# StuLiu/RegDA

Measured on AMD Instinct MI355X. Metric: src+tgt 512x512 image-pairs/sec (SSL step), higher is better.
Workload: dtype bf16; 1 GPU; st.regda.2potsdam SSL step, resnet101 DeepLabV2(PPM), batch 8+8 512x512 per GPU, online EMA teacher; global_batch=8, parallelism=dp1

## Files before the change

include/rgda_hip.h:

```cpp
#ifndef RGDA_HIP_H
#define RGDA_HIP_H

#include <stddef.h>
#include <stdint.h>

#ifdef __cplusplus
extern "C" {
#endif

#define RGDA_ABI_VERSION 10
#define RGDA_STAT_REPLICAS 8
#define RGDA_STAT_FRAC_FWD 26
#define RGDA_STAT_FRAC_BWD 40
typedef int64_t rgda_stat_t;
#define RGDA_LAYOUT_TILE 64

typedef void* rgda_stream_t;

enum rgda_status {
    RGDA_OK = 0,
    RGDA_ERR_ARG = -1,
    RGDA_ERR_WORKSPACE = -2,
    RGDA_ERR_LAUNCH = -3,
    RGDA_ERR_UNSUPPORTED = -4
// ... 138 lines not shown
    int lddw, co_split;
} rgda_wgrad_desc;
size_t rgda_conv2d_wgrad_workspace(const rgda_wgrad_desc* descs, int n);
const char* rgda_conv2d_wgrad_kernel(const rgda_wgrad_desc* desc);
int rgda_conv2d_wgrad_grouped(const rgda_wgrad_desc* descs, int n, void* ws, size_t ws_bytes, rgda_stream_t stream);

int rgda_stem_im2col(const float* img, void* col, int N, int H, int W, int Ho, int Wo, int Kp,
                     rgda_stream_t stream);

int rgda_stem_conv(const float* img, const void* wgt, void* y, int ldy, rgda_stat_t* stats, int stat_groups, int N,
                   int H, int W, int Ho, int Wo, rgda_stream_t stream);
int rgda_stem_conv_bneval(const float* img, const void* wgt, void* y, int ldy, const float* running_mean,
                          const float* running_var, const float* gamma, const float* beta, float eps, int relu,
                          int N, int H, int W, int Ho, int Wo, rgda_stream_t stream);

int rgda_bn_stats(const void* x, int ldx, rgda_stat_t* stats, int64_t M, int C, rgda_stream_t stream);
int rgda_bn_finalize(const rgda_stat_t* stats, float* mi, float* running_mean, float* running_var,
                     int64_t* num_batches_tracked, int64_t M, int C, int groups, float eps,
                     float momentum, rgda_stream_t stream);
int rgda_bn_apply(const void* x, int ldx, const float* mi, const float* gamma, const float* beta,
                  const void* res, int ldres, const float* nscale, int rows_per_image, void* y,
                  int ldy, int64_t M, int C, int relu, int groups, rgda_stream_t stream);
int rgda_bn_train_apply(const void* x, int ldx, const rgda_stat_t* stats, float* mi, float* running_mean,
                        float* running_var, int64_t* num_batches_tracked, const float* gamma,
                        const float* beta, const void* res, int ldres, const float* nscale,
                        int rows_per_image, void* y, int ldy, uint8_t* relu_mask, int64_t M, int C, int relu,
                        int groups, float eps, float momentum, rgda_stream_t stream);
int rgda_bn_bwd_reduce(const void* g, int ldg, const void* y, int ldy, const uint8_t* relu_mask, const void* x,
                       int ldx, const float* mi, const float* nscale, int rows_per_image, rgda_stat_t* sums,
                       int64_t M, int C, int relu, const float* gamma, const float* beta, int groups,
                       rgda_stream_t stream);
int rgda_bn_bwd_apply(const void* g, int ldg, const void* y, int ldy, const uint8_t* relu_mask, const void* x,
                      int ldx, const float* mi, const float* gamma, const float* nscale,
                      int rows_per_image, const rgda_stat_t* sums, void* dx, int lddx, void* gmask,
                      int ldgm, float* dgamma, float* dbeta, int64_t M, int C, int relu, const float* beta,
                      void* act_out, int ldact, int groups, rgda_stream_t stream);

typedef struct rgda_bn_small_fwd_desc {
    const void* x; void* y; uint8_t* relu_mask; const float* gamma; const float* beta; float* mi;
    float* running_mean; float* running_var; int64_t* num_batches_tracked;
    int64_t M; int ldx, ldy, C, groups, relu; float eps, momentum;
} rgda_bn_small_fwd_desc;
typedef struct rgda_bn_small_bwd_desc {
    const void* g; const void* y; const uint8_t* relu_mask; const void* x; void* dx; const float* mi; const float* gamma;
    float* dgamma; float* dbeta;
    int64_t M; int ldg, ldy, ldx, lddx, C, groups, relu;
} rgda_bn_small_bwd_desc;
int rgda_bn_train_small(const rgda_bn_small_fwd_desc* descs, int n, rgda_stream_t stream);
int rgda_bn_bwd_small(const rgda_bn_small_bwd_desc* descs, int n, rgda_stream_t stream);

int rgda_maxpool_fwd(const void* x, void* y, uint8_t* idx, int N, int H, int W, int C, int Ho,
                     int Wo, rgda_stream_t stream);
int rgda_maxpool_bwd(const void* gy, const uint8_t* idx, void* gx, int N, int H, int W, int C,
                     int Ho, int Wo, rgda_stream_t stream);
int rgda_maxpool_fwd_bnin(const rgda_bn_operand* bn_in, const void* x, void* y, uint8_t* idx, int N, int H, int W,
                          int C, int Ho, int Wo, rgda_stream_t stream);

int rgda_instnorm_fwd(const void* x, int ldx, void* y0, void* y1, int ldy, float* feat_nchw,
                      float* mi, int N, int HW, int C, float eps, rgda_stream_t stream);
int rgda_instnorm_bwd(const void* ga, const void* gb, int ldg, const void* gc, int ldgc,
                      const void* x, int ldx, const float* mi, void* dx, int lddx, int N, int HW,
                      int C, rgda_stream_t stream);

int rgda_spatial_mix(const void* in, int ldin, const float* Mx, void* out, int ldout, int N, int I,
                     int J, int C, int accumulate, int out_f32, rgda_stream_t stream);

int rgda_spatial_mix_multi(int nsrc, const void* const* ins, const int* ldins, const float* const* mats,
                           const int* Js, void* out, int ldout, int N, int I, int C, rgda_stream_t stream);

int rgda_classifier_fwd(const void* hidden, int ldh, const float* w, const float* bias,
                        float* logits, int N, int HW, int C, int ncls, rgda_stream_t stream);
size_t rgda_classifier_bwd_workspace(int64_t M, int C, int ncls);
int rgda_classifier_bwd(const void* hidden, int ldh, const float* w, const float* glogits,
                        void* dhidden, int lddh, float* dw, float* db, int N, int HW, int C,
                        int ncls, void* ws, size_t ws_bytes, rgda_stream_t stream);


int rgda_sumsq(const float* g, int64_t n, float* out, float* ws, rgda_stream_t stream);

int rgda_sgd_step(float* p, const float* g, float* v, float* shadow, void* p_bf16, void* shadow_bf16,
                  const float* gnorm_sq, const float* lr_dev, int64_t n, float momentum,
                  float weight_decay, float max_norm, float gscale, float ema_decay,
                  int first_step, rgda_stream_t stream);

size_t rgda_stem_wgrad_workspace(int N, int H, int W);
int rgda_stem_wgrad(const float* img, const void* dy, int lddy, float* dw, void* ws, size_t ws_bytes, int N, int H,
                    int W, int Ho, int Wo, rgda_stream_t stream);

int rgda_weight_transpose_bf16(const float* w, void* wt, int Co, int T, int Ci, rgda_stream_t stream);
int rgda_weight_transpose_batched(const int64_t* table, int n, int64_t total_blocks, rgda_stream_t stream);
int rgda_cast_bf16(const float* src, void* dst, int64_t n, rgda_stream_t stream);
int rgda_cast_f32(const void* src_bf16, float* dst, int64_t n, rgda_stream_t stream);
int rgda_ddp_accumulate_bf16(const void* recv, int world, void* out, int64_t shard_elems, rgda_stream_t stream);

typedef void* rgda_comm_t;
#define RGDA_COMM_ID_BYTES 128
#define RGDA_COMM_F32 0
#define RGDA_COMM_BF16 1
#define RGDA_COMM_I64 2
#define RGDA_COMM_F64 3
int rgda_comm_unique_id(void* id_128_bytes);
int rgda_comm_init(const void* id_128_bytes, int rank, int world, rgda_comm_t* comm);
int rgda_comm_destroy(rgda_comm_t comm);
int rgda_comm_all_reduce(rgda_comm_t comm, void* buf, int64_t n, int dtype, rgda_stream_t stream);
int rgda_comm_all_gather(rgda_comm_t comm, const void* send, void* recv, int64_t n_per_rank, int dtype,
                         rgda_stream_t stream);
int rgda_comm_all_to_all(rgda_comm_t comm, const void* send, void* recv, int64_t n_per_rank, int dtype,
                         rgda_stream_t stream);
int rgda_pad_cast_bf16(const float* src, void* dst, int R, int K, int Kp, rgda_stream_t stream);
int rgda_unpad_acc_f32(const float* src, float* dst, int R, int K, int Kp, rgda_stream_t stream);
int rgda_fill_zero(void* p, size_t bytes, rgda_stream_t stream);
int rgda_copy_multi(int n, void* const* dsts, const void* const* srcs, const size_t* bytes, rgda_stream_t stream);
int rgda_set_f32(float* p, float value, rgda_stream_t stream);
int rgda_dropout_mask(float* out, int64_t n, float p, uint64_t seed, rgda_stream_t stream);
int rgda_add_bf16(const void* a, int lda, const void* b, int ldb, void* out, int ldo, int64_t M,
                  int C, rgda_stream_t stream);


int rgda_dihedral_nchw(const float* src, float* dst, int N, int C, int Hs, int Ws, int hflip, int rot_k,
                       int flip_first, float scale, int accumulate, rgda_stream_t stream);

int rgda_pad_rows_nchw(const float* src, float* dst, int N, int C, int h, int w, int top, int bottom,
                       rgda_stream_t stream);
int rgda_window_crop(const float* full, float* tile, int N, int C, int Hf, int Wf, int y1, int x1, int h, int w,
                     int Th, int Tw, rgda_stream_t stream);
int rgda_window_accumulate(const float* tile, float* full, float* count, int N, int C, int Hf, int Wf, int y1,
                           int x1, int h, int w, int Th, int Tw, rgda_stream_t stream);
int rgda_window_normalise(float* full, const float* count, int N, int C, int Hf, int Wf, rgda_stream_t stream);

int rgda_window_gather(const float* src_f32, const uint8_t* src_u8, const float* lut, const int32_t* windows, int K,
                       int views, int n, int C, int H, int W, int Th, int Tw, float* out, int* flag,
                       rgda_stream_t stream);
int rgda_window_scatter(const float* pred, const int32_t* windows, int K, int views, int n, int C, int H, int W, int Th,
                        int Tw, int row0, int rows, float* full, float* count, int* flag, rgda_stream_t stream);
int rgda_window_finish(float* full, const float* count, int n, int C, int H, int W, uint8_t* labels_u8,
                       int64_t* labels_i64, const int64_t* y_true, int64_t* cm, int* flag, rgda_stream_t stream);

int rgda_resize_bilinear_ac(const float* src, float* dst, int N, int C, int h, int w, int H, int W,
                            rgda_stream_t stream);


int rgda_augment_tiles(const uint8_t* img, const uint8_t* label, const float* soft, const int32_t* regs,
                       const int32_t* params, int N, int Hi, int Wi, int C, int Ho, int Wo, const float* lut,
                       const int32_t* label_lut, float* img_out, int64_t* label_out, float* soft_out, int64_t* regs_out,
                       int* flag, rgda_stream_t stream);


size_t rgda_superpixels_workspace(int N, int H, int W, int S);
int rgda_superpixels(const uint8_t* img, int N, int H, int W, int S, int m, int iters, int min_area, int32_t* regs_out,
                     int32_t* count_out, void* ws, size_t ws_bytes, rgda_stream_t stream);

int rgda_region_shrink(const int32_t* regs, int N, int H, int W, int win, int fill, int32_t* out, rgda_stream_t stream);


int rgda_argmax_nchw(const float* probs, int64_t* out, int N, int C, int64_t HW, rgda_stream_t stream);
int rgda_confusion_accumulate(const int64_t* y_true, const int64_t* y_pred, int64_t* cm, int* flag, int64_t n,
                              int C, rgda_stream_t stream);


size_t rgda_pcl_loss_workspace(int C, int K);
int rgda_pcl_loss(const float* feat, const int64_t* labels, const float* protos, float* loss, void* dfeat,
                  int lddf, int accumulate, int b, int K, int C, int h, int w, int ignore_label,
                  float temperature, float weight, void* ws, size_t ws_bytes, rgda_stream_t stream);

size_t rgda_coral_loss_workspace(int ns, int nt, int d);
int rgda_coral_loss(const float* feat_s, int bs, int hws, int64_t ldcs, int64_t ldbs,
// ... 36 lines not shown
```

regda_amd/csrc/optim_kernels.hip:

```cpp
#include "common.h"

__global__ void __launch_bounds__(256) sumsq_partial_kernel(const float* __restrict__ g, long long n, float* part) {
    double acc = 0.0;
    long long n4 = n >> 2;
    const float4* g4 = (const float4*)g;
    for (long long i = (long long)blockIdx.x * 256 + threadIdx.x; i < n4; i += (long long)gridDim.x * 256) {
        float4 v = g4[i];
        acc += (double)(v.x * v.x + v.y * v.y) + (double)(v.z * v.z + v.w * v.w);
    }
    if (blockIdx.x == 0 && threadIdx.x < (n & 3)) { float v = g[(n4 << 2) + threadIdx.x]; acc += (double)v * v; }
    __shared__ double red[256];
    red[threadIdx.x] = acc;
    __syncthreads();
    for (int o = 128; o > 0; o >>= 1) {
        if (threadIdx.x < o) red[threadIdx.x] += red[threadIdx.x + o];
        __syncthreads();
    }
    if (threadIdx.x == 0) part[blockIdx.x] = (float)red[0];
}
__global__ void __launch_bounds__(256) sumsq_final_kernel(const float* __restrict__ part, int n, float* out) {
    __shared__ double red[256];
    double acc = 0.0;
    for (int i = threadIdx.x; i < n; i += 256) acc += part[i];
    red[threadIdx.x] = acc;
    __syncthreads();
    for (int o = 128; o > 0; o >>= 1) {
        if (threadIdx.x < o) red[threadIdx.x] += red[threadIdx.x + o];
        __syncthreads();
    }
    if (threadIdx.x == 0) out[0] = (float)red[0];
}

extern "C" int rgda_sumsq(const float* g, int64_t n, float* out, float* ws, rgda_stream_t stream) {
    if (!g || !out || !ws || n <= 0) return RGDA_ERR_ARG;
    hipStream_t st = to_stream(stream);
    int blocks = min(cdiv(n, 256 * 16), 1024);
    sumsq_partial_kernel<<<blocks, 256, 0, st>>>(g, n, ws);
    RGDA_CHECK_LAUNCH();
    sumsq_final_kernel<<<1, 256, 0, st>>>(ws, blocks, out);
    RGDA_CHECK_LAUNCH();
    return RGDA_OK;
}

__global__ void __launch_bounds__(256) sgd_step_kernel(float* __restrict__ p, const float* __restrict__ g,
                                                       float* __restrict__ v, float* __restrict__ shadow,
                                                       bf16_t* __restrict__ pb, bf16_t* __restrict__ sb,
                                                       const float* __restrict__ gnorm_sq,
                                                       const float* __restrict__ lr_dev, long long n4, float momentum,
                                                       float wd, float max_norm, float gscale, float ema_d,
                                                       int first_step) {
    const float total = sqrtf(gnorm_sq[0]) * gscale;
    const float coef = fminf(max_norm / (total + 1e-6f), 1.f) * gscale;
    const float lr = lr_dev[0];
    float4* p4 = (float4*)p;
    const float4* g4 = (const float4*)g;
    float4* v4 = (float4*)v;
    float4* s4 = (float4*)shadow;
    for (long long i = (long long)blockIdx.x * 256 + threadIdx.x; i < n4; i += (long long)gridDim.x * 256) {
        float4 pp = p4[i], gg = g4[i], vv;
        float d0 = gg.x * coef + wd * pp.x, d1 = gg.y * coef + wd * pp.y, d2 = gg.z * coef + wd * pp.z,
              d3 = gg.w * coef + wd * pp.w;
        if (first_step) { vv = make_float4(d0, d1, d2, d3); }
        else {
            vv = v4[i];
            vv.x = momentum * vv.x + d0; vv.y = momentum * vv.y + d1; vv.z = momentum * vv.z + d2; vv.w = momentum * vv.w + d3;
        }
        pp.x -= lr * vv.x; pp.y -= lr * vv.y; pp.z -= lr * vv.z; pp.w -= lr * vv.w;
        v4[i] = vv;
        p4[i] = pp;
        if (shadow) {
            float4 ss = s4[i];
            const float a = 1.f - ema_d;
            ss.x = a * pp.x + ema_d * ss.x; ss.y = a * pp.y + ema_d * ss.y; ss.z = a * pp.z + ema_d * ss.z; ss.w = a * pp.w + ema_d * ss.w;
            s4[i] = ss;
            if (sb) {
                uint2 pk;
                pk.x = pack2bf(ss.x, ss.y);
                pk.y = pack2bf(ss.z, ss.w);
                *(uint2*)(sb + (i << 2)) = pk;
            }
        }
        if (pb) {
            uint2 pk;
            pk.x = pack2bf(pp.x, pp.y);
            pk.y = pack2bf(pp.z, pp.w);
            *(uint2*)(pb + (i << 2)) = pk;
        }
    }
}

extern "C" int rgda_sgd_step(float* p, const float* g, float* v, float* shadow, void* p_bf16, void* shadow_bf16, const float* gnorm_sq,
                             const float* lr_dev, int64_t n, float momentum, float weight_decay, float max_norm,
                             float gscale, float ema_decay, int first_step, rgda_stream_t stream) {
    if (!p || !g || !v || !gnorm_sq || !lr_dev || n <= 0 || (n & 3)) return RGDA_ERR_ARG;
    long long n4 = n >> 2;
    int blocks = min(cdiv(n4, 256 * 4), 4096);
    sgd_step_kernel<<<blocks, 256, 0, to_stream(stream)>>>(p, g, v, shadow, (bf16_t*)p_bf16, (bf16_t*)shadow_bf16, gnorm_sq, lr_dev, n4,
                                                            momentum, weight_decay, max_norm, gscale, ema_decay,
                                                            first_step);
    RGDA_CHECK_LAUNCH();
    return RGDA_OK;
}

__global__ void __launch_bounds__(256) cast_bf16_kernel(const float* __restrict__ src, bf16_t* __restrict__ dst, long long n) {
    long long n4 = n >> 2;
    const float4* s4 = (const float4*)src;
    for (long long i = (long long)blockIdx.x * 256 + threadIdx.x; i < n4; i += (long long)gridDim.x * 256) {
        float4 v = s4[i];
        uint2 pk;
        pk.x = pack2bf(v.x, v.y);
        pk.y = pack2bf(v.z, v.w);
        *(uint2*)(dst + (i << 2)) = pk;
    }
    if (blockIdx.x == 0 && threadIdx.x < (n & 3)) dst[(n4 << 2) + threadIdx.x] = f2bf(src[(n4 << 2) + threadIdx.x]);
}

extern "C" int rgda_cast_bf16(const float* src, void* dst, int64_t n, rgda_stream_t stream) {
    if (!src || !dst || n <= 0) return RGDA_ERR_ARG;
    int blocks = min(cdiv(n, 256 * 16), 4096);
    cast_bf16_kernel<<<blocks, 256, 0, to_stream(stream)>>>(src, (bf16_t*)dst, n);
    RGDA_CHECK_LAUNCH();
    return RGDA_OK;
}

__global__ void __launch_bounds__(256) ddp_accumulate_bf16_kernel(const bf16_t* __restrict__ recv, int world, bf16_t* __restrict__ out,
                                                                  long long s) {
    const long long nv = s >> 3;
    for (long long i = (long long)blockIdx.x * 256 + threadIdx.x; i < nv; i += (long long)gridDim.x * 256) {
        float acc[8] = {0.f, 0.f, 0.f, 0.f, 0.f, 0.f, 0.f, 0.f};
        for (int r = 0; r < world; ++r) {
            const u16x8 v = *(const u16x8*)(recv + (size_t)r * s + i * 8);
#pragma unroll
            for (int e = 0; e < 8; ++e) acc[e] += bf2f(v[e]);
        }
        uint4 pk;
        pk.x = pack2bf(acc[0], acc[1]); pk.y = pack2bf(acc[2], acc[3]); pk.z = pack2bf(acc[4], acc[5]); pk.w = pack2bf(acc[6], acc[7]);
        *(uint4*)(out + i * 8) = pk;
    }
}

extern "C" int rgda_ddp_accumulate_bf16(const void* recv, int world, void* out, int64_t shard_elems, rgda_stream_t stream) {
    if (!recv || !out || world < 1 || shard_elems <= 0 || (shard_elems & 7)) return RGDA_ERR_ARG;
    const int blocks = min(cdiv(shard_elems >> 3, 256), 2048);
    ddp_accumulate_bf16_kernel<<<blocks, 256, 0, to_stream(stream)>>>((const bf16_t*)recv, world, (bf16_t*)out, shard_elems);
    RGDA_CHECK_LAUNCH();
    return RGDA_OK;
}

__global__ void __launch_bounds__(256) cast_f32_kernel(const bf16_t* __restrict__ src, float* __restrict__ dst, long long n) {
    for (long long i = (long long)blockIdx.x * 256 + threadIdx.x; i < n; i += (long long)gridDim.x * 256) dst[i] = bf2f(src[i]);
}

extern "C" int rgda_cast_f32(const void* src, float* dst, int64_t n, rgda_stream_t stream) {
    if (!src || !dst || n <= 0) return RGDA_ERR_ARG;
    cast_f32_kernel<<<min(cdiv(n, 256 * 8), 4096), 256, 0, to_stream(stream)>>>((const bf16_t*)src, dst, n);
    RGDA_CHECK_LAUNCH();
    return RGDA_OK;
}

__global__ void __launch_bounds__(256) weight_transpose_kernel(const float* __restrict__ w, bf16_t* __restrict__ wt, int Co,
                                                               int T, int Ci) {
    __shared__ float tile[32][33];
    const int tap = blockIdx.z, co0 = blockIdx.y * 32, ci0 = blockIdx.x * 32;
    const int tx = threadIdx.x & 31, ty = threadIdx.x >> 5;
    for (int r = ty; r < 32; r += 8) {
        int co = co0 + r, ci = ci0 + tx;
        tile[r][tx] = (co < Co && ci < Ci) ? w[((size_t)co * T + tap) * Ci + ci] : 0.f;
    }
    __syncthreads();
    for (int r = ty; r < 32; r += 8) {
        int ci = ci0 + r, co = co0 + tx;
        if (ci < Ci && co < Co) wt[((size_t)ci * T + tap) * Co + co] = f2bf(tile[tx][r]);
    }
}

__global__ void __launch_bounds__(256) weight_transpose_batched_kernel(const long long* __restrict__ table, int n) {
    constexpr int TS = RGDA_LAYOUT_TILE;
    __shared__ float tile[TS][TS + 1];
    constexpr int NFB = 1024;
    __shared__ long long fb[NFB];
    const long long b = blockIdx.x;
    int lo = 0, hi = n - 1;
    if (n <= NFB) {
        for (int i = threadIdx.x; i < n; i += 256) fb[i] = table[i * 8 + 5];
        __syncthreads();
// ... 213 lines not shown
```

regda_amd/ops.py:

```python
import ctypes

import torch

from ._lib import lib


MIN_CLASSES, MAX_CLASSES = 6, 16


def check_class_count(c, who='class_num'):
    if not MIN_CLASSES <= int(c) <= MAX_CLASSES:
        raise ValueError(f'{who}: {c} classes; the kernels serve {MIN_CLASSES} <= class_num <= {MAX_CLASSES}')


_LDS_LOSS_ROW, _LDS_PCL, _LDS_REFINE = 0, 1, 2


def check_step_shape(c, k, H, W, who='step'):
    check_class_count(c, who)
    L = lib()
    w = (int(W) + 15) // 16
    row, lim = L.size('rgda_class_lds', _LDS_LOSS_ROW, c, w, W), L.size('rgda_class_lds_limit', _LDS_LOSS_ROW)
    if row > lim:
        raise ValueError(f'{who}: {c} classes at {W}-pixel rows need {row} B of LDS in the fused upsample + loss row pass, '
# ... 615 lines not shown
    lib().call('rgda_maxpool_fwd', x.data_ptr(), y.data_ptr(), idx.data_ptr(), N, H, W, C, Ho, Wo, _stream())


def maxpool_fwd_bnin(bnop, x, y, idx, N, H, W, C, Ho, Wo):
    lib().call('rgda_maxpool_fwd_bnin', bnop, x.data_ptr(), y.data_ptr(), idx.data_ptr(), N, H, W, C, Ho, Wo, _stream())


def maxpool_bwd(gy, idx, gx, N, H, W, C, Ho, Wo):
    lib().call('rgda_maxpool_bwd', gy.data_ptr(), idx.data_ptr(), gx.data_ptr(), N, H, W, C, Ho, Wo, _stream())


def instnorm_fwd(x, y0, y1, feat, mi, N, HW, C, eps=1e-5):
    ldy = _ld(y0) if y0 is not None else (_ld(y1) if y1 is not None else 0)
    lib().call('rgda_instnorm_fwd', x.data_ptr(), _ld(x), _p(y0), _p(y1), ldy, _p(feat), mi.data_ptr(), N, HW, C, eps,
               _stream())


def instnorm_bwd(ga, gb, gc, x, mi, dx, N, HW, C):
    ldg = _ld(ga) if ga is not None else (_ld(gb) if gb is not None else 0)
    lib().call('rgda_instnorm_bwd', _p(ga), _p(gb), ldg, _p(gc), _ld(gc) if gc is not None else 0, x.data_ptr(),
               _ld(x), mi.data_ptr(), dx.data_ptr(), _ld(dx), N, HW, C, _stream())


def spatial_mix_multi(ins, mats, out, N, I, C):
    import ctypes
    n = len(ins)
    P = (ctypes.c_void_p * n)(*[t.data_ptr() for t in ins])
    L = (ctypes.c_int * n)(*[_ld(t) for t in ins])
    Mt = (ctypes.c_void_p * n)(*[m.data_ptr() for m in mats])
    J = (ctypes.c_int * n)(*[m.shape[1] for m in mats])
    for m in mats:
        assert m.shape[0] == I and m.is_contiguous() and m.dtype == torch.float32
    lib().call('rgda_spatial_mix_multi', n, P, L, Mt, J, out.data_ptr(), _ld(out), N, I, C, _stream())


def spatial_mix(inp, Mx, out, N, I, J, C, accumulate=False):
    assert Mx.shape == (I, J) and Mx.is_contiguous() and Mx.dtype == torch.float32
    lib().call('rgda_spatial_mix', inp.data_ptr(), _ld(inp), Mx.data_ptr(), out.data_ptr(), _ld(out), N, I, J, C,
               int(accumulate), int(out.dtype == torch.float32), _stream())


def group_mix(inp, W, out, G, I, J, C):
    assert W.shape == (I, J) and W.is_contiguous() and W.dtype == torch.float32
    assert inp.shape[0] == G * J and out.shape[0] == G * I
    lib().call('rgda_group_mix', inp.data_ptr(), _ld(inp), int(inp.dtype == torch.float32), W.data_ptr(),
               out.data_ptr(), _ld(out), int(out.dtype == torch.float32), G, I, J, C, _stream())


def sparse_mix(ins, csr, outs, N, C):
    import ctypes
    rowptr, cols, vals = csr
    outs = [outs] if torch.is_tensor(outs) else list(outs)
    assert rowptr.dtype == torch.int32 and cols.dtype == torch.int32 and vals.dtype == torch.float32
    rows = [o.shape[0] // N for o in outs]
    assert rowptr.numel() == sum(rows) + 1 and all(o.shape[0] == N * r for o, r in zip(outs, rows))
    n, m = len(ins), len(outs)
    P = (ctypes.c_void_p * n)(*[t.data_ptr() for t in ins])
    L = (ctypes.c_int * n)(*[_ld(t) for t in ins])
    J = (ctypes.c_int * n)(*[t.shape[0] // N for t in ins])
    O = (ctypes.c_void_p * m)(*[t.data_ptr() for t in outs])
    OL = (ctypes.c_int * m)(*[_ld(t) for t in outs])
    OR = (ctypes.c_int * m)(*rows)
    lib().call('rgda_sparse_mix', n, P, L, J, int(ins[0].dtype == torch.float32), rowptr.data_ptr(), cols.data_ptr(),
               vals.data_ptr(), m, O, OL, OR, int(outs[0].dtype == torch.float32), N, C, _stream())


def classifier_fwd(hidden, w, bias, logits, N, HW, C, ncls):
    lib().call('rgda_classifier_fwd', hidden.data_ptr(), _ld(hidden), w.data_ptr(), bias.data_ptr(), logits.data_ptr(),
               N, HW, C, ncls, _stream())


def classifier_bwd(hidden, w, glogits, dhidden, dw, db, N, HW, C, ncls):
    L = lib()
    ws = _ws(L.size('rgda_classifier_bwd_workspace', N * HW, C, ncls), hidden.device)
    L.call('rgda_classifier_bwd', hidden.data_ptr(), _ld(hidden), w.data_ptr(), glogits.data_ptr(),
           dhidden.data_ptr(), _ld(dhidden), dw.data_ptr(), db.data_ptr(), N, HW, C, ncls, ws.data_ptr(), ws.numel(),
           _stream())


def sumsq(g, out, ws):
    lib().call('rgda_sumsq', g.data_ptr(), g.numel(), out.data_ptr(), ws.data_ptr(), _stream())


def sgd_step(p, g, v, shadow, p_bf16, gnorm_sq, lr_dev, momentum, weight_decay, max_norm, gscale, ema_decay,
             first_step, shadow_bf16=None):
    lib().call('rgda_sgd_step', p.data_ptr(), g.data_ptr(), v.data_ptr(), _p(shadow), _p(p_bf16), _p(shadow_bf16),
               gnorm_sq.data_ptr(),
               lr_dev.data_ptr(), p.numel(), momentum, weight_decay, max_norm, gscale, ema_decay, int(first_step),
               _stream())


def weight_transpose_bf16(w, wt, Co, T, Ci):
    lib().call('rgda_weight_transpose_bf16', w.data_ptr(), wt.data_ptr(), Co, T, Ci, _stream())


def weight_transpose_batched(table, n, total_blocks):
    lib().call('rgda_weight_transpose_batched', table.data_ptr(), n, total_blocks, _stream())


def cast_bf16(src, dst):
    lib().call('rgda_cast_bf16', src.data_ptr(), dst.data_ptr(), src.numel(), _stream())


def cast_f32(src, dst):
    lib().call('rgda_cast_f32', src.data_ptr(), dst.data_ptr(), dst.numel(), _stream())


def ddp_accumulate_bf16(recv, world, out):
    lib().call('rgda_ddp_accumulate_bf16', recv.data_ptr(), world, out.data_ptr(), out.numel(), _stream())


def pad_cast_bf16(src, dst, R, K, Kp):
    lib().call('rgda_pad_cast_bf16', src.data_ptr(), dst.data_ptr(), R, K, Kp, _stream())


def unpad_acc_f32(src, dst, R, K, Kp):
    lib().call('rgda_unpad_acc_f32', src.data_ptr(), dst.data_ptr(), R, K, Kp, _stream())


def add_bf16(a, b, out, M, C):
    lib().call('rgda_add_bf16', a.data_ptr(), _ld(a), b.data_ptr(), _ld(b), out.data_ptr(), _ld(out), M, C, _stream())


def dihedral(src, hflip, k, flip_first, dst=None, scale=1.0, accumulate=False):
    _need_cuda(src)
    n, c, h, w = src.shape
    k = k % 4
    ho, wo = (w, h) if (k & 1) else (h, w)
    if dst is None:
        assert not accumulate
        dst = torch.empty(n, c, ho, wo, device=src.device)
    assert src.is_contiguous() and dst.is_contiguous() and src.dtype == dst.dtype == torch.float32
    assert tuple(dst.shape) == (n, c, ho, wo)
    lib().call('rgda_dihedral_nchw', src.data_ptr(), dst.data_ptr(), n, c, h, w, int(bool(hflip)), k, int(bool(flip_first)),
               float(scale), int(bool(accumulate)), _stream())
    return dst


def window_crop(full, y1, x1, h, w, Th, Tw):
    n, c, Hf, Wf = full.shape
    tile = torch.empty(n, c, Th, Tw, device=full.device)
    lib().call('rgda_window_crop', full.data_ptr(), tile.data_ptr(), n, c, Hf, Wf, y1, x1, h, w, Th, Tw, _stream())
    return tile


def window_accumulate(tile, full, count, y1, x1, h, w):
    n, c, Hf, Wf = full.shape
    lib().call('rgda_window_accumulate', tile.data_ptr(), full.data_ptr(), count.data_ptr(), n, c, Hf, Wf, y1, x1, h, w,
               tile.shape[2], tile.shape[3], _stream())


def window_normalise(full, count):
    n, c, Hf, Wf = full.shape
    lib().call('rgda_window_normalise', full.data_ptr(), count.data_ptr(), n, c, Hf, Wf, _stream())


def window_gather(src, windows, tile, views=1, lut=None, out=None, flag=None):
    _need_cuda(src, windows, lut, out, flag)
    th, tw = tile
    if src.dtype == torch.uint8:
        n, H, W, c = src.shape
        if c != 3 or lut is None:
            raise ValueError('window_gather: a uint8 source is [n][H][W][3] and needs lut')
        f32, u8 = None, src.contiguous()
    else:
        if src.dtype != torch.float32 or src.dim() != 4:
            raise ValueError('window_gather: the source is f32 [n][C][H][W] or uint8 [n][H][W][3]')
        n, c, H, W = src.shape
# ... 267 lines not shown
```

regda_amd/ssl.py:

```python
import torch

from . import ops
from . import plan
from .ddp import FlatGradReducer, all_reduce_prototype_statistics
from .gast.balance import source_loss, target_loss


class SSLStep:
    def __init__(self, model, prototypes, class_num=6, ignore_label=-1, momentum=0.9, weight_decay=5e-4,
                 max_norm=32.0, cutoff_top=0.8, cutoff_low=0.6, percent=0.5, proto_decay=0.996, refine_temp=2.0,
                 sam_refine=True, refine_label=True, ema_decay=None, max_regions=4096, bucket_elems=12 << 20,
                 process_group=None, overlap_wgrad=True, overlap_comm=True, class_balancer_s=None,
                 class_balancer_t=None, grad_payload='fp32', comm=None, loss_s='CrossEntropy', loss_t='none',
                 uvem_m=0.2, uvem_t=0.7, uvem_g=4.0):
        ops.check_class_count(class_num, type(self).__name__)
        self.model = model
        self.C, self.ig = class_num, ignore_label
        self._shape_ok = None
        self.momentum, self.wd, self.max_norm = momentum, weight_decay, max_norm
        self.top, self.low, self.percent = cutoff_top, cutoff_low, percent
        self.pdecay, self.temp = proto_decay, refine_temp
        self.sam_refine, self.refine_label = sam_refine, refine_label
        self.max_regions = max_regions
        dev = model.device
        self.prototypes = prototypes.to(dev).float().contiguous().clone()
        self.mom = torch.zeros_like(model.flat_p)
        self.lr_dev = torch.zeros(1, device=dev)
        self.gn = torch.zeros(1, device=dev)
        self.gn_ws = torch.zeros(1024, device=dev)
        self.first = True
        self.lrh_ws = None
        self.ema_decay = ema_decay
        self.teacher = None
        if ema_decay is not None:
            self.teacher = model.make_teacher()
        bounds = model.param_boundaries()
        self.comm = comm
        self.reducer = FlatGradReducer(model.flat_g, bounds, bucket_elems, process_group, payload=grad_payload, comm=comm)
        self.measure_comm = False
        self.comm_events = None
        self.bwd_start_event = None
        self.wgrad_stream = torch.cuda.Stream(device=dev) if overlap_wgrad else None
        self.source_side = overlap_wgrad
        self.class_balancer_s, self.class_balancer_t = class_balancer_s, class_balancer_t
        self.loss_fn_s = source_loss(loss_s, class_balancer_s, ignore_label)
        self.loss_fn_t = target_loss(loss_t, class_balancer_t, uvem_m, uvem_t, uvem_g, class_num, ignore_label,
                                     device=dev)
        self._graph = None
        self._plan = None
        self._proto_ready = None
        self.proto_stats = None
        self.marks = None
        self.overlap_comm = overlap_comm
        self.keep_debug = False
        self.debug = None
        self.world = self.reducer.world
        self.group = process_group

    @torch.no_grad()
    def step(self, images_s, label_s, images_t, soft_t, regs_t, lr):
        self._check_shape(images_s, images_t)
        if self._graph is not None:
            return self._replay(images_s, label_s, images_t, soft_t, regs_t, lr)
        if self._plan is not None:
            return self._replay_plan(images_s, label_s, images_t, soft_t, regs_t, lr)
        ops.set_f32(self.lr_dev, lr)
        with ops.use_stream(torch.cuda.current_stream()):
            return self._step(images_s, label_s, images_t, soft_t, regs_t)

    def _check_shape(self, *images):
        for x in images:
            if x is None or tuple(x.shape[-2:]) == self._shape_ok:
                continue
            ops.check_step_shape(self.C, self.prototypes.shape[-1], x.shape[-2], x.shape[-1], type(self).__name__)
            self._shape_ok = tuple(x.shape[-2:])

    def capture(self, images_s, label_s, images_t, soft_t, regs_t):
        self._check_shape(images_s, images_t)
        assert not self.first, 'run one eager step before capture()'
        if self.world > 1:
            raise RuntimeError('whole-step graphs are single-GPU; the multi-GPU path stays eager')
        if self._host_balancers():
            raise RuntimeError('class balancing (--bcs / --bct) is host-side state: use record_plan(), not capture()')
        self._static = self._static_inputs(images_s, label_s, images_t, soft_t, regs_t)
        torch.cuda.synchronize()
        m = self.model
        m._hw_ready = m._wt_ready = None
        g = torch.cuda.CUDAGraph()
        with torch.cuda.graph(g):
            with ops.use_stream(torch.cuda.current_stream()):
                self._out = self._step(*self._static)
                if self.wgrad_stream is not None:
                    torch.cuda.current_stream().wait_stream(self.wgrad_stream)
        m._hw_ready = m._wt_ready = None
        self._graph = g

    @staticmethod
    def _static_inputs(images_s, label_s, images_t, soft_t, regs_t):
        conv = lambda t, dt: None if t is None else t.detach().to(dt).contiguous().clone()
        return [conv(images_s, torch.float32), conv(label_s, torch.int64), conv(images_t, torch.float32),
                conv(soft_t, torch.float32), conv(regs_t, torch.int64)]

    def teacher_model(self):
        t = self.teacher
        if t is None:
            return None
        t.adopt_buffers(self.model)
        t.refresh_from_master(mirror_is_fresh=(not self.first) and t.flat_p._version == t._synced_version)
        t.eval()
        return t

    def record_plan(self, images_s, label_s, images_t, soft_t, regs_t, lr=None):
# ... 108 lines not shown
        self._mark('student forward done')
        s1, t1, s2, t2 = x1[:nb], x1[nb:], x2[:nb], x2[nb:]
        g1, g2 = torch.empty_like(x1), torch.empty_like(x2)
        feat_s, feat_t = feat[:nb], feat[nb:]
        if teacher_on_side:
            plan.wait_stream(main, self.wgrad_stream)
        elif online:
            soft_t = self.teacher_probs(images_t, snapshot=False)
        self.last_soft_t = soft_t
        self._mark('joined teacher')
        def wait_prototypes():
            if self._proto_ready is not None:
                main.wait_event(self._proto_ready)
                self._proto_ready = None
        plan.host(wait_prototypes)
        side = self.wgrad_stream if self.source_side else None
        if side is not None:
            plan.wait_event(side, plan.record_event(main))
            with ops.use_stream(side):
                loss_s = self._source_loss(s1, s2, label_s, g1[:nb], g2[:nb])
        regs = (regs_t.squeeze(1) if regs_t.dim() == 4 else regs_t) if self.sam_refine else None
        fuse_lrh = (self.refine_label and self.sam_refine and not self.keep_debug and self.max_regions <= 65535
                    and (soft_t.shape[-1] * soft_t.shape[-2]) % 4 == 0)
        hard = None
        if self.refine_label:
            soft, cm = ops.label_refine(feat_t, self.prototypes, t1, t2, soft_t, self.temp, return_ws=True)
            if not fuse_lrh:
                hard = ops.pseudo_select(soft, self.top, self.low, self.ig, classmax_ws=cm, check=False)
        else:
            soft = soft_t
            hard = ops.pseudo_select(soft_t, self.top, self.low, self.ig, check=False)
        exchange_protos = self.reducer.active
        if side is not None:
            plan.wait_event(side, plan.record_event(main))
            with ops.use_stream(side):
                self._proto_local(feat_s, label_s, exchange_protos)
            source_done = plan.record_event(side)
        if self.keep_debug:
            self.debug = dict(t1=t1, t2=t2, s1=s1, s2=s2, feat_t=feat_t, feat_s=feat_s, soft_in=soft_t, soft=soft,
                              hard_selected=hard)
        if self.sam_refine:
            self._lrh_flag_off = (regs.shape[0] * self.max_regions * (self.C + 1)) * 4
            if fuse_lrh:
                hard, self.lrh_ws = ops.pseudo_lrh(soft, cm, regs, self.top, self.low, self.percent, self.C, self.ig,
                                                   self.max_regions, ws=self.lrh_ws)
            else:
                need = self._lrh_flag_off + 16
                if self.lrh_ws is None or self.lrh_ws.numel() < need:
                    self.lrh_ws = torch.empty(need, dtype=torch.uint8, device=m.device)
                hard = ops.lrh(hard, regs.contiguous(), self.percent, self.C, self.ig, self.max_regions, check=False,
                               ws=self.lrh_ws)
        if side is None:
            self._proto_local(feat_s, label_s, exchange_protos)
        if exchange_protos:
            pside = self.wgrad_stream if self.wgrad_stream is not None else main
            if pside is not main and side is None:
                plan.wait_event(pside, plan.record_event(main))
            def exchange_statistics():
                all_reduce_prototype_statistics(self.proto_stats, self.C, self.prototypes.shape[1], self.group, self.comm,
                                                world=self.world)
            with ops.use_stream(pside):
                plan.host(exchange_statistics)
                ops.proto_apply(self.prototypes, self.proto_stats, self.pdecay)
                plan.host(lambda: setattr(self, '_proto_ready', pside.record_event() if pside is not main else None))
        if side is None:
            loss_s = self._source_loss(s1, s2, label_s, g1[:nb], g2[:nb])
        loss_t = self._target_loss(t1, t2, hard, soft, g1[nb:], g2[nb:])
        if side is not None:
            plan.wait_event(main, source_done)
        self._mark('label path + losses done')
        self._inputs_done = plan.record_event(main)
        self._backward_and_update(T, main, g1, g2)
        self.last_hard = hard
        return loss_s, loss_t, self.gn

    def _proto_local(self, feat_s, label_s, exchange):
        if exchange:
            self.proto_stats, _ = ops.proto_stats(feat_s, label_s, 16, self.ig, 0.75, self.C, stats=self.proto_stats)
        else:
            ops.proto_update(feat_s, label_s, self.prototypes, 16, self.ig, 0.75, self.pdecay)

    def _backward_and_update(self, T, main, g1, g2, gfeat=None):
        m = self.model
        plan.host(self.reducer.reset)
        if self.measure_comm and self.reducer.active:
            def mark_backward_start():
                self.reducer.measure = True
                self.bwd_start_event = torch.cuda.Event(enable_timing=True)
                self.bwd_start_event.record()
            plan.host(mark_backward_start)
        T['wgrad_stream'] = self.wgrad_stream
        T['main_stream'] = main
        T['mark'] = self._mark if self.marks is not None else None

        def progress(offset):
            if (self.world > 1 or self.reducer.force) and self.overlap_comm:
                if self.wgrad_stream is not None:
                    plan.wait_event(self.wgrad_stream, plan.record_event(main))
                    with ops.use_stream(self.wgrad_stream):
                        plan.host(lambda: self.reducer.ready_down_to(offset))
                else:
                    plan.host(lambda: self.reducer.ready_down_to(offset))
        m._backward_plan(T, g1, g2, on_progress=progress, gfeat=gfeat)
        self._mark('backward done (streams joined)')
        def finish_exchange():
            if self.measure_comm and self.reducer.active:
                e0, e1 = torch.cuda.Event(enable_timing=True), torch.cuda.Event(enable_timing=True)
                e0.record()
                self.reducer.finish()
                e1.record()
                self.comm_events = (e0, e1)
            else:
                self.reducer.finish()
        plan.host(finish_exchange)
        ops.sumsq(m.flat_g, self.gn, self.gn_ws)
        shadow = self.teacher.flat_p if self.teacher is not None else None
        ops.sgd_step(m.flat_p, m.flat_g, self.mom, shadow, m.flat_pb, self.gn, self.lr_dev, self.momentum, self.wd,
                     self.max_norm, self.reducer.gscale, self.ema_decay if shadow is not None else 0.0, self.first,
                     shadow_bf16=self.teacher.flat_pb if shadow is not None else None)
        self.first = False
        m.sync_derived_weights(self.wgrad_stream)
        m._synced_version = m.flat_p._version
        self._mark('optimizer + weight mirrors done')

    @torch.no_grad()
    def teacher_probs(self, images_t, snapshot=True):
        t = self.teacher
        if snapshot:
            t.adopt_buffers(self.model)
        t.refresh_from_master(mirror_is_fresh=(t.flat_p._version == t._synced_version))
        t.eval()
        x1, x2, _ = t._forward_plan(images_t.contiguous().float(), None)
        return ops.teacher_probs(x1, x2, tuple(images_t.shape[-2:]))

    def lrh_flag(self):
        if self.lrh_ws is None:
            return 0
        o = self._lrh_flag_off
        return int(self.lrh_ws[o:o + 4].view(torch.int32).item())
```

Baseline: 451.0 pairs/s.

## Overlap gradient-norm reduction with backward via per-segment sumsq accumulation

When no DDP reducer is active, the squared gradient norm is computed in segments as backward progresses, on the wgrad stream, and accumulated into a float64 device scalar instead of one full pass over flat_g after backward. The SGD step reads the accumulated norm directly and gains a slab-partitioned, optionally unrolled launch with a larger grid, with FMA-explicit arithmetic. This removes a full serial read of the gradient buffer from the critical path. It adds many small kernel launches and extra cross-stream event waits during backward, and the final SGD kernel now depends on the wgrad stream having finished the segments.

```diff
diff --git a/include/rgda_hip.h b/include/rgda_hip.h
--- a/include/rgda_hip.h
+++ b/include/rgda_hip.h
@@ -244,6 +244,13 @@
                   const float* gnorm_sq, const float* lr_dev, int64_t n, float momentum,
                   float weight_decay, float max_norm, float gscale, float ema_decay,
                   int first_step, rgda_stream_t stream);
+
+int rgda_sumsq_segment(const float* g, int64_t n, double* acc, float* ws, rgda_stream_t stream);
+
+int rgda_sgd_step_acc(float* p, const float* g, float* v, float* shadow, void* p_bf16, void* shadow_bf16,
+                      const double* gnorm_acc, float* gnorm_out, const float* lr_dev, int64_t n, float momentum,
+                      float weight_decay, float max_norm, float gscale, float ema_decay,
+                      int first_step, rgda_stream_t stream);
 
 size_t rgda_stem_wgrad_workspace(int N, int H, int W);
 int rgda_stem_wgrad(const float* img, const void* dy, int lddy, float* dw, void* ws, size_t ws_bytes, int N, int H,
diff --git a/regda_amd/csrc/optim_kernels.hip b/regda_amd/csrc/optim_kernels.hip
--- a/regda_amd/csrc/optim_kernels.hip
+++ b/regda_amd/csrc/optim_kernels.hip
@@ -42,65 +42,192 @@
     return RGDA_OK;
 }
 
+__device__ __forceinline__ double block_sum_f64(double acc) {
+    __shared__ double red[256];
+    red[threadIdx.x] = acc;
+    __syncthreads();
+    for (int o = 128; o > 0; o >>= 1) {
+        if (threadIdx.x < o) red[threadIdx.x] += red[threadIdx.x + o];
+        __syncthreads();
+    }
+    return red[0];
+}
+__global__ void __launch_bounds__(256) sumsq_segment_kernel(const float* __restrict__ g, long long n, double* __restrict__ part,
+                                                            double* __restrict__ acc_out) {
+    const long long head = min(n, (long long)((4 - (((uintptr_t)g >> 2) & 3)) & 3));
+    const long long n4 = (n - head) >> 2, tail0 = head + (n4 << 2);
+    const float4* g4 = (const float4*)(g + head);
+    double acc = 0.0;
+    for (long long i = (long long)blockIdx.x * 256 + threadIdx.x; i < n4; i += (long long)gridDim.x * 256) {
+        const float4 v = g4[i];
+        acc += ((double)v.x * v.x + (double)v.y * v.y) + ((double)v.z * v.z + (double)v.w * v.w);
+    }
+    if (blockIdx.x == 0) {
+        if ((long long)threadIdx.x < head) { const double v = g[threadIdx.x]; acc += v * v; }
+        if (tail0 + threadIdx.x < n && threadIdx.x < 4) { const double v = g[tail0 + threadIdx.x]; acc += v * v; }
+    }
+    const double s = block_sum_f64(acc);
+    if (threadIdx.x == 0) {
+        if (gridDim.x == 1) acc_out[0] += s;
+        else part[blockIdx.x] = s;
+    }
+}
+__global__ void __launch_bounds__(256) sumsq_segment_final_kernel(const double* __restrict__ part, int n, double* __restrict__ acc_out) {
+    double acc = 0.0;
+    for (int i = threadIdx.x; i < n; i += 256) acc += part[i];
+    const double s = block_sum_f64(acc);
+    if (threadIdx.x == 0) acc_out[0] += s;
+}
+
+extern "C" int rgda_sumsq_segment(const float* g, int64_t n, double* acc, float* ws, rgda_stream_t stream) {
+    if (!g || !acc || !ws || n <= 0 || ((uintptr_t)g & 3) || ((uintptr_t)acc & 7) || ((uintptr_t)ws & 7)) return RGDA_ERR_ARG;
+    hipStream_t st = to_stream(stream);
+    const int blocks = (int)min((long long)cdiv(n, 256 * 16), 1024ll);
+    sumsq_segment_kernel<<<blocks, 256, 0, st>>>(g, n, (double*)ws, acc);
+    RGDA_CHECK_LAUNCH();
+    if (blocks > 1) {
+        sumsq_segment_final_kernel<<<1, 256, 0, st>>>((const double*)ws, blocks, acc);
+        RGDA_CHECK_LAUNCH();
+    }
+    return RGDA_OK;
+}
+
+template <int U>
 __global__ void __launch_bounds__(256) sgd_step_kernel(float* __restrict__ p, const float* __restrict__ g,
                                                        float* __restrict__ v, float* __restrict__ shadow,
                                                        bf16_t* __restrict__ pb, bf16_t* __restrict__ sb,
-                                                       const float* __restrict__ gnorm_sq,
-                                                       const float* __restrict__ lr_dev, long long n4, float momentum,
-                                                       float wd, float max_norm, float gscale, float ema_d,
+                                                       const float* __restrict__ gnorm_sq, const double* __restrict__ gnorm_acc,
+                                                       float* __restrict__ gnorm_out,
+                                                       const float* __restrict__ lr_dev, long long n4, long long per,
+                                                       float momentum, float wd, float max_norm, float gscale, float ema_d,
                                                        int first_step) {
-    const float total = sqrtf(gnorm_sq[0]) * gscale;
-    const float coef = fminf(max_norm / (total + 1e-6f), 1.f) * gscale;
-    const float lr = lr_dev[0];
+    const float gn = gnorm_acc ? (float)gnorm_acc[0] : gnorm_sq[0];
+    if (gnorm_out && blockIdx.x == 0 && threadIdx.x == 0) gnorm_out[0] = gn;
+    const float coef = __fmul_rn(fminf(max_norm / __fmaf_rn(gscale, sqrtf(gn), 1e-6f), 1.f), gscale);
+    const float lr = lr_dev[0], nlr = -lr;
+    const float a = 1.f - ema_d;
     float4* p4 = (float4*)p;
     const float4* g4 = (const float4*)g;
     float4* v4 = (float4*)v;
     float4* s4 = (float4*)shadow;
-    for (long long i = (long long)blockIdx.x * 256 + threadIdx.x; i < n4; i += (long long)gridDim.x * 256) {
-        float4 pp = p4[i], gg = g4[i], vv;
-        float d0 = gg.x * coef + wd * pp.x, d1 = gg.y * coef + wd * pp.y, d2 = gg.z * coef + wd * pp.z,
-              d3 = gg.w * coef + wd * pp.w;
-        if (first_step) { vv = make_float4(d0, d1, d2, d3); }
-        else {
-            vv = v4[i];
-            vv.x = momentum * vv.x + d0; vv.y = momentum * vv.y + d1; vv.z = momentum * vv.z + d2; vv.w = momentum * vv.w + d3;
-        }
-        pp.x -= lr * vv.x; pp.y -= lr * vv.y; pp.z -= lr * vv.z; pp.w -= lr * vv.w;
-        v4[i] = vv;
-        p4[i] = pp;
-        if (shadow) {
-            float4 ss = s4[i];
-            const float a = 1.f - ema_d;
-            ss.x = a * pp.x + ema_d * ss.x; ss.y = a * pp.y + ema_d * ss.y; ss.z = a * pp.z + ema_d * ss.z; ss.w = a * pp.w + ema_d * ss.w;
-            s4[i] = ss;
-            if (sb) {
+    long long i0 = (long long)blockIdx.x * 256 + threadIdx.x, end = n4, stride = (long long)gridDim.x * 256;
+    if (per) {
+        i0 = (long long)blockIdx.x * per + threadIdx.x;
+        end = min(n4, ((long long)blockIdx.x + 1) * per);
+        stride = 256;
+    }
+    for (; i0 < end; i0 += stride * U) {
+        float4 pp[U], gg[U], vv[U], ss[U];
+#pragma unroll
+        for (int u = 0; u < U; ++u) {
+            const long long i = i0 + u * stride;
+            if (i < end) {
+                pp[u] = p4[i];
+                gg[u] = g4[i];
+                if (!first_step) vv[u] = v4[i];
+                if (shadow) ss[u] = s4[i];
+            }
+        }
+#pragma unroll
+        for (int u = 0; u < U; ++u) {
+            const long long i = i0 + u * stride;
+            if (i >= end) continue;
+            float4 P = pp[u], V;
+            const float d0 = __fmaf_rn(wd, P.x, __fmul_rn(gg[u].x, coef)), d1 = __fmaf_rn(wd, P.y, __fmul_rn(gg[u].y, coef)),
+                        d2 = __fmaf_rn(wd, P.z, __fmul_rn(gg[u].z, coef)), d3 = __fmaf_rn(wd, P.w, __fmul_rn(gg[u].w, coef));
+            if (first_step) { V = make_float4(d0, d1, d2, d3); }
+            else {
+                V = vv[u];
+                V.x = __fmaf_rn(momentum, V.x, d0); V.y = __fmaf_rn(momentum, V.y, d1);
+                V.z = __fmaf_rn(momentum, V.z, d2); V.w = __fmaf_rn(momentum, V.w, d3);
+            }
+            P.x = __fmaf_rn(nlr, V.x, P.x); P.y = __fmaf_rn(nlr, V.y, P.y); P.z = __fmaf_rn(nlr, V.z, P.z); P.w = __fmaf_rn(nlr, V.w, P.w);
+            v4[i] = V;
+            p4[i] = P;
+            if (shadow) {
+                float4 S = ss[u];
+                S.x = __fmaf_rn(a, P.x, __fmul_rn(ema_d, S.x)); S.y = __fmaf_rn(a, P.y, __fmul_rn(ema_d, S.y));
+                S.z = __fmaf_rn(a, P.z, __fmul_rn(ema_d, S.z)); S.w = __fmaf_rn(a, P.w, __fmul_rn(ema_d, S.w));
+                s4[i] = S;
+                if (sb) {
+                    uint2 pk;
+                    pk.x = pack2bf(S.x, S.y);
+                    pk.y = pack2bf(S.z, S.w);
+                    *(uint2*)(sb + (i << 2)) = pk;
+                }
+            }
+            if (pb) {
                 uint2 pk;
-                pk.x = pack2bf(ss.x, ss.y);
-                pk.y = pack2bf(ss.z, ss.w);
-                *(uint2*)(sb + (i << 2)) = pk;
+                pk.x = pack2bf(P.x, P.y);
+                pk.y = pack2bf(P.z, P.w);
+                *(uint2*)(pb + (i << 2)) = pk;
             }
         }
-        if (pb) {
-            uint2 pk;
-            pk.x = pack2bf(pp.x, pp.y);
-            pk.y = pack2bf(pp.z, pp.w);
-            *(uint2*)(pb + (i << 2)) = pk;
-        }
-    }
+    }
+}
+
+static constexpr int SGD_U = 1, SGD_GRID = 8192, SGD_SLAB = 1;
+
+static int sgd_step_launch(float* p, const float* g, float* v, float* shadow, void* p_bf16, void* shadow_bf16, const float* gnorm_sq,
+                           const double* gnorm_acc, float* gnorm_out, const float* lr_dev, int64_t n, float momentum,
+                           float weight_decay, float max_norm, float gscale, float ema_decay, int first_step, rgda_stream_t stream) {
+    if (!p || !g || !v || (!gnorm_sq && !gnorm_acc) || !lr_dev || n <= 0 || (n & 3)) return RGDA_ERR_ARG;
+    const long long n4 = n >> 2;
+    int U = SGD_U, grid = SGD_GRID, slab = SGD_SLAB;
+    if (const char* e = TUNE_ENV("RGDA_SGD_U")) U = atoi(e);
+    if (const char* e = TUNE_ENV("RGDA_SGD_GRID")) grid = atoi(e);
+    if (const char* e = TUNE_ENV("RGDA_SGD_SLAB")) slab = atoi(e);
+    if ((U != 1 && U != 2 && U != 4) || grid < 1) return RGDA_ERR_ARG;
+    const int blocks = (int)min((long long)cdiv(n4, 256 * U), (long long)grid);
+    const long long per = slab ? (long long)cdiv(cdiv(n4, blocks), 256) * 256 : 0;
+#define RGDA_SGD_LAUNCH(UU)                                                                                                     \
+    sgd_step_kernel<UU><<<blocks, 256, 0, to_stream(stream)>>>(p, g, v, shadow, (bf16_t*)p_bf16, (bf16_t*)shadow_bf16, gnorm_sq,  \
+                                                               gnorm_acc, gnorm_out, lr_dev, n4, per, momentum, weight_decay,    \
+                                                               max_norm, gscale, ema_decay, first_step)
+    if (U == 1) RGDA_SGD_LAUNCH(1);
+    else if (U == 2) RGDA_SGD_LAUNCH(2);
+    else RGDA_SGD_LAUNCH(4);
+#undef RGDA_SGD_LAUNCH
+    RGDA_CHECK_LAUNCH();
+    return RGDA_OK;
 }
 
 extern "C" int rgda_sgd_step(float* p, const float* g, float* v, float* shadow, void* p_bf16, void* shadow_bf16, const float* gnorm_sq,
                              const float* lr_dev, int64_t n, float momentum, float weight_decay, float max_norm,
                              float gscale, float ema_decay, int first_step, rgda_stream_t stream) {
-    if (!p || !g || !v || !gnorm_sq || !lr_dev || n <= 0 || (n & 3)) return RGDA_ERR_ARG;
-    long long n4 = n >> 2;
-    int blocks = min(cdiv(n4, 256 * 4), 4096);
-    sgd_step_kernel<<<blocks, 256, 0, to_stream(stream)>>>(p, g, v, shadow, (bf16_t*)p_bf16, (bf16_t*)shadow_bf16, gnorm_sq, lr_dev, n4,
-                                                            momentum, weight_decay, max_norm, gscale, ema_decay,
-                                                            first_step);
-    RGDA_CHECK_LAUNCH();
-    return RGDA_OK;
-}
+    if (!gnorm_sq) return RGDA_ERR_ARG;
+    return sgd_step_launch(p, g, v, shadow, p_bf16, shadow_bf16, gnorm_sq, nullptr, nullptr, lr_dev, n, momentum, weight_decay,
+                           max_norm, gscale, ema_decay, first_step, stream);
+}
+
+extern "C" int rgda_sgd_step_acc(float* p, const float* g, float* v, float* shadow, void* p_bf16, void* shadow_bf16,
+                                 const double* gnorm_acc, float* gnorm_out, const float* lr_dev, int64_t n, float momentum,
+                                 float weight_decay, float max_norm, float gscale, float ema_decay, int first_step,
+                                 rgda_stream_t stream) {
+    if (!gnorm_acc) return RGDA_ERR_ARG;
+    return sgd_step_launch(p, g, v, shadow, p_bf16, shadow_bf16, nullptr, gnorm_acc, gnorm_out, lr_dev, n, momentum, weight_decay,
+                           max_norm, gscale, ema_decay, first_step, stream);
+}
+
+#ifdef RGDA_TUNING
+__global__ void __launch_bounds__(256) copy9_kernel(float4* __restrict__ p, const float4* __restrict__ g, float4* __restrict__ v,
+                                                    float4* __restrict__ s, uint2* __restrict__ pb, uint2* __restrict__ sb, long long n4) {
+    for (long long i = (long long)blockIdx.x * 256 + threadIdx.x; i < n4; i += (long long)gridDim.x * 256) {
+        const float4 a = p[i], b = g[i], c = v[i], d = s[i];
+        v[i] = b; p[i] = c; s[i] = a;
+        pb[i] = make_uint2(__float_as_uint(d.x), __float_as_uint(d.y));
+        sb[i] = make_uint2(__float_as_uint(d.z), __float_as_uint(d.w));
+    }
+}
+extern "C" int rgda_tune_copy9(float* p, const float* g, float* v, float* s, void* pb, void* sb, int64_t n, int grid,
+                               rgda_stream_t stream) {
+    if (!p || !g || !v || !s || !pb || !sb || n <= 0 || (n & 3) || grid < 1) return RGDA_ERR_ARG;
+    copy9_kernel<<<grid, 256, 0, to_stream(stream)>>>((float4*)p, (const float4*)g, (float4*)v, (float4*)s, (uint2*)pb, (uint2*)sb,
+                                                      n >> 2);
+    RGDA_CHECK_LAUNCH();
+    return RGDA_OK;
+}
+#endif
 
 __global__ void __launch_bounds__(256) cast_bf16_kernel(const float* __restrict__ src, bf16_t* __restrict__ dst, long long n) {
     long long n4 = n >> 2;
diff --git a/regda_amd/ops.py b/regda_amd/ops.py
--- a/regda_amd/ops.py
+++ b/regda_amd/ops.py
@@ -721,8 +721,18 @@
     lib().call('rgda_sumsq', g.data_ptr(), g.numel(), out.data_ptr(), ws.data_ptr(), _stream())
 
 
+def sumsq_segment(g, acc, ws):
+    assert g.dtype == torch.float32 and acc.dtype == torch.float64 and ws.numel() * ws.element_size() >= 8192
+    lib().call('rgda_sumsq_segment', g.data_ptr(), g.numel(), acc.data_ptr(), ws.data_ptr(), _stream())
+
+
 def sgd_step(p, g, v, shadow, p_bf16, gnorm_sq, lr_dev, momentum, weight_decay, max_norm, gscale, ema_decay,
-             first_step, shadow_bf16=None):
+             first_step, shadow_bf16=None, gnorm_acc=None):
+    if gnorm_acc is not None:
+        lib().call('rgda_sgd_step_acc', p.data_ptr(), g.data_ptr(), v.data_ptr(), _p(shadow), _p(p_bf16), _p(shadow_bf16),
+                   gnorm_acc.data_ptr(), _p(gnorm_sq), lr_dev.data_ptr(), p.numel(), momentum, weight_decay, max_norm,
+                   gscale, ema_decay, int(first_step), _stream())
+        return
     lib().call('rgda_sgd_step', p.data_ptr(), g.data_ptr(), v.data_ptr(), _p(shadow), _p(p_bf16), _p(shadow_bf16),
                gnorm_sq.data_ptr(),
                lr_dev.data_ptr(), p.numel(), momentum, weight_decay, max_norm, gscale, ema_decay, int(first_step),
diff --git a/regda_amd/ssl.py b/regda_amd/ssl.py
--- a/regda_amd/ssl.py
+++ b/regda_amd/ssl.py
@@ -27,7 +27,9 @@
         self.mom = torch.zeros_like(model.flat_p)
         self.lr_dev = torch.zeros(1, device=dev)
         self.gn = torch.zeros(1, device=dev)
-        self.gn_ws = torch.zeros(1024, device=dev)
+        self.gn_ws = torch.zeros(2048, device=dev)
+        self.gn_acc = torch.zeros(2, dtype=torch.float64, device=dev)
+        self.norm_cover = None
         self.first = True
         self.lrh_ws = None
         self.ema_decay = ema_decay
@@ -302,6 +304,16 @@
 
     def _backward_and_update(self, T, main, g1, g2, gfeat=None):
         m = self.model
+        segmented = not self.reducer.active
+        cover, hi = [], [m.flat_g.numel()]
+        if segmented:
+            ops.fill_zero(self.gn_acc)
+
+        def norm_segment(lo):
+            if lo < hi[0]:
+                ops.sumsq_segment(m.flat_g[lo:hi[0]], self.gn_acc, self.gn_ws)
+                cover.append((lo, hi[0]))
+                hi[0] = lo
         plan.host(self.reducer.reset)
         if self.measure_comm and self.reducer.active:
             def mark_backward_start():
@@ -314,6 +326,16 @@
         T['mark'] = self._mark if self.marks is not None else None
 
         def progress(offset):
+            if segmented:
+                if offset >= hi[0]:
+                    return
+                if self.wgrad_stream is not None:
+                    plan.wait_event(self.wgrad_stream, plan.record_event(main))
+                    with ops.use_stream(self.wgrad_stream):
+                        norm_segment(offset)
+                else:
+                    norm_segment(offset)
+                return
             if (self.world > 1 or self.reducer.force) and self.overlap_comm:
                 if self.wgrad_stream is not None:
                     plan.wait_event(self.wgrad_stream, plan.record_event(main))
@@ -333,11 +355,18 @@
             else:
                 self.reducer.finish()
         plan.host(finish_exchange)
-        ops.sumsq(m.flat_g, self.gn, self.gn_ws)
+        if segmented:
+            norm_segment(0)
+            assert hi[0] == 0 and sum(b - a for a, b in cover) == m.flat_g.numel() and \
+                all(cover[i][0] == cover[i + 1][1] for i in range(len(cover) - 1)), 'norm segments do not partition flat_g'
+            self.norm_cover = cover
+        else:
+            ops.sumsq(m.flat_g, self.gn, self.gn_ws)
         shadow = self.teacher.flat_p if self.teacher is not None else None
         ops.sgd_step(m.flat_p, m.flat_g, self.mom, shadow, m.flat_pb, self.gn, self.lr_dev, self.momentum, self.wd,
                      self.max_norm, self.reducer.gscale, self.ema_decay if shadow is not None else 0.0, self.first,
-                     shadow_bf16=self.teacher.flat_pb if shadow is not None else None)
+                     shadow_bf16=self.teacher.flat_pb if shadow is not None else None,
+                     gnorm_acc=self.gn_acc if segmented else None)
         self.first = False
         m.sync_derived_weights(self.wgrad_stream)
         m._synced_version = m.flat_p._version
```

New measurement: 451.0 pairs/s (median of 2 runs). Within noise of the previous version (-0.0%).
